# Tonmoy1321/Multimodal-DeepFake-Detection

Measured on AMD Instinct MI355X. Metric: clips/sec (node) XceptionLSTMV 16x299x299 bf16 train, higher is better.
Workload: dtype bf16; 1 GPU; XceptionLSTMV(hidden=128) unfrozen-backbone train step, 16 clips/GPU x 16 frames x 3x299x299, BCE + clip 1.0 + Adam; global_batch=16, frames=16, size=299, mode=unfrozen, optimizer=clip 1.0 + Adam, xcp FusedAdamClip, parallelism=dp1, execution=eager launches

## Files before the change

### include/xcp.h

```cpp
#ifndef XCP_H_
#define XCP_H_

#ifdef __cplusplus
extern "C" {
#endif

typedef void* xcp_stream_t;

#define XCP_OK 0
#define XCP_EINVAL 1001
#define XCP_EUNSUPPORTED 1002
#define XCP_F32 0
#define XCP_BF16 1
#define XCP_ACT_NONE 0
#define XCP_ACT_RELU 1
#define XCP_ACT_BNRELU 2

int xcp_gemm_nt(int dtype, const void* A, long lda, const void* B, long ldb, void* C, long ldc, int M, int N, int K,
                float* stats, int gmode, int gH, int gW, int gOH, int gOW, int gS, int gC, int tile, xcp_stream_t stream);
int xcp_gemm_nt_stat_rows(int M);

int xcp_gemm_tn_rows_per_split(int dtype, int gmode, int M, int N, int K, int tile);
int xcp_gemm_tn(int dtype, const void* G, long ldg, const void* X, long ldx, float* P, int M, int N, int K, int S,
                int rows_per_split, int gmode, int gH, int gW, int gOH, int gOW, int gS, int gC, int tile,
// ... 13 lines not shown
int xcp_dw_bwd(int dtype, int act, const void* dY, const void* X, const float* Wt, const float* scale, const float* shift,
               const void* dRes, const void* dSkip, int sOH, int sOW, int sS, int skip_pre, void* dX, float* dWpart,
               float* bnpart, const float* bmean, const float* binvstd, int N, int H, int W, int C,
               xcp_stream_t stream);
int xcp_dw_bwd_resbn(int dtype, int act, const void* dY, const void* X, const float* Wt, const float* scale,
                     const float* shift, const void* dRes, void* dX, float* dWpart, float* bnpart, const float* bmean,
                     const float* binvstd, const void* Yb, int N, int H, int W, int C, xcp_stream_t stream);

int xcp_colreduce_f32(const float* in, int S, long L, long ld, float* out, int G, int accumulate, xcp_stream_t stream);
int xcp_colreduce_multi(const long long* jobs, int njobs, xcp_stream_t stream);
int xcp_colreduce_groups(int S, long L);
int xcp_chanred_parts(long rows, int C);
int xcp_row_stats(int dtype, const void* X, long rows, int C, float* part, xcp_stream_t stream);
int xcp_bn_bwd_reduce(int dtype, const void* dZ, const void* Y, const float* mean, const float* invstd,
                      const float* ms, const float* mt, long rows, int C, float* part, xcp_stream_t stream);
int xcp_bn_finalize_part(const float* part, int R, int C, int CP, double count, const float* gamma, const float* beta,
                         float* rmean, float* rvar, float momentum, float eps, float* mean_o, float* invstd_o,
                         float* scale_o, float* shift_o, xcp_stream_t stream);
#define XCP_FIN_ACCUMULATE 1
#define XCP_FIN_NARROW 2
int xcp_bn_bwd_finalize_part(const float* part, int R, int C, int CP, double count, const float* gamma,
                             const float* mean, const float* invstd, float* alpha, float* bcoef, float* delta,
                             float* dgamma, float* dbeta, int flags, xcp_stream_t stream);
int xcp_bn_finalize(const double* part2, int G, int C, int CP, double count, const float* gamma, const float* beta,
                    float* rmean, float* rvar, float momentum, float eps, int train, float* mean, float* invstd,
                    float* scale, float* shift, xcp_stream_t stream);
int xcp_bn_act(int dtype, const void* X, void* Y, const float* scale, const float* shift, int relu, long rows, int C,
               xcp_stream_t stream);
int xcp_bn_act_strided(int dtype, const void* X, void* Y, const float* scale, const float* shift, int relu, int N, int H,
                       int W, int OH, int OW, int S, int C, xcp_stream_t stream);
int xcp_bn_bwd_apply(int dtype, const void* dZ, const void* Y, void* dY, const float* alpha, const float* bcoef,
                     const float* delta, const float* ms, const float* mt, long rows, int C, xcp_stream_t stream);
int xcp_relu_bwd(int dtype, void* dX, const void* X, long rows, int C, xcp_stream_t stream);
int xcp_tail_fwd(int dtype, const void* Y, const float* s1, const float* t1, int pool, const void* S, const float* s2,
                 const float* t2, void* Out, unsigned char* amax, int N, int H, int W, int C, xcp_stream_t stream);
int xcp_maxpool_bwd(int dtype, const void* dOut, const unsigned char* amax, void* dZ, int N, int H, int W, int C,
                    xcp_stream_t stream);
int xcp_maxpool_bwd_bnred_parts(int N, int H, int W, int C);
int xcp_maxpool_bwd_bnred(int dtype, const void* dOut, const unsigned char* amax, void* dZ, const void* Y,
                          const float* mean, const float* invstd, int N, int H, int W, int C, float* part,
                          xcp_stream_t stream);
int xcp_avgpool_fwd(int dtype, const void* Y, const float* s, const float* t, float* F, int N, int HW, int C,
                    xcp_stream_t stream);
int xcp_avgpool_bwd(int dtype, const float* dF, const void* Y, const float* s, const float* t, void* dZ, int N, int HW,
                    int C, xcp_stream_t stream);

int xcp_conv1_fwd(int dtype, const float* X, const float* W, void* Y, int N, int IH, int IW, xcp_stream_t stream);
// ... 63 lines not shown
```

### multimodal-deepfake-detection_amd/xcp/_lib.py

```python
import ctypes
import os

_HERE = os.path.dirname(os.path.abspath(__file__))
LIB_PATH = DEFAULT_LIB_PATH = os.path.join(_HERE, "libxcp.so")
_REPO = os.path.dirname(os.path.dirname(_HERE))
_OVERRIDE = os.environ.get("XCP_LIB_PATH")
if _OVERRIDE:
    _real = os.path.realpath(_OVERRIDE)
    if os.path.commonpath([_real, os.path.realpath(_REPO)]) != os.path.realpath(_REPO):
        raise ImportError(f"XCP_LIB_PATH={_OVERRIDE} is outside the repository ({_REPO}); "
                          "only in-tree A/B builds may replace libxcp.so")
    LIB_PATH = _real
MISSING = []

P = ctypes.c_void_p
I = ctypes.c_int
L = ctypes.c_long
F = ctypes.c_float
D = ctypes.c_double

SIGNATURES = {
    "xcp_gemm_nt": [I, P, L, P, L, P, L, I, I, I, P, I, I, I, I, I, I, I, I, P],
    "xcp_gemm_nt_stat_rows": [I],
    "xcp_gemm_tn_rows_per_split": [I, I, I, I, I, I],
    "xcp_gemm_tn": [I, P, L, P, L, P, I, I, I, I, I, I, I, I, I, I, I, I, I, P],
    "xcp_unit_bwd_rows_per_split": [I, I, I, I],
    "xcp_unit_bwd": [I, P, P, P, P, P, P, P, P, P, I, I, I, I, I, P],
    "xcp_dw_fwd": [I, I, P, P, P, P, P, I, I, I, I, P],
    "xcp_sep_fwd_parts": [I, I, I, I, I, I],
    "xcp_sep_fwd": [I, I, P, P, P, P, P, P, P, P, I, I, I, I, I, P],
    "xcp_dw_bwd_chunks": [I, I, I, I],
    "xcp_dw_bwd": [I, I, P, P, P, P, P, P, P, I, I, I, I, P, P, P, P, P, I, I, I, I, P],
    "xcp_dw_bwd_resbn": [I, I, P, P, P, P, P, P, P, P, P, P, P, P, I, I, I, I, P],
    "xcp_colreduce_f32": [P, I, L, L, P, I, I, P],
    "xcp_colreduce_groups": [I, L],
    "xcp_colreduce_multi": [P, I, P],
    "xcp_chanred_parts": [L, I],
    "xcp_row_stats": [I, P, L, I, P, P],
    "xcp_bn_bwd_reduce": [I, P, P, P, P, P, P, L, I, P, P],
    "xcp_bn_finalize_part": [P, I, I, I, D, P, P, P, P, F, F, P, P, P, P, P],
    "xcp_bn_bwd_finalize_part": [P, I, I, I, D, P, P, P, P, P, P, P, P, I, P],
    "xcp_bn_finalize": [P, I, I, I, D, P, P, P, P, F, F, I, P, P, P, P, P],
    "xcp_bn_act": [I, P, P, P, P, I, L, I, P],
    "xcp_bn_act_strided": [I, P, P, P, P, I, I, I, I, I, I, I, I, P],
    "xcp_bn_bwd_apply": [I, P, P, P, P, P, P, P, P, L, I, P],
    "xcp_relu_bwd": [I, P, P, L, I, P],
    "xcp_tail_fwd": [I, P, P, P, I, P, P, P, P, P, I, I, I, I, P],
    "xcp_maxpool_bwd": [I, P, P, P, I, I, I, I, P],
    "xcp_maxpool_bwd_bnred_parts": [I, I, I, I],
    "xcp_maxpool_bwd_bnred": [I, P, P, P, P, P, P, I, I, I, I, P, P],
    "xcp_avgpool_fwd": [I, P, P, P, P, I, I, I, P],
    "xcp_avgpool_bwd": [I, P, P, P, P, P, I, I, I, P],
    "xcp_conv1_fwd": [I, P, P, P, I, I, I, P],
    "xcp_conv1_fwd_parts": [I, I, I],
    "xcp_conv1_fwd_stats": [I, P, P, P, P, I, I, I, P],
    "xcp_conv1_wgrad_parts": [I, I, I],
    "xcp_conv1_wgrad": [I, P, P, P, I, I, I, P],
    "xcp_conv1_wgrad_fused": [I, I, I],
    "xcp_conv1_wgrad_bn": [I, P, P, P, P, P, P, P, P, P, I, I, I, P],
    "xcp_permute3": [I, P, P, I, I, I, I, I, I, P],
# ... 73 lines not shown
```

### multimodal-deepfake-detection_amd/xcp/csrc/bn.hip

```cpp
#include "common.h"

namespace {

template <bool ACC, int VEC>
__global__ __launch_bounds__(256) void colreduce_kernel(const float* __restrict__ in, int S, long L, long ld,
                                                        float* __restrict__ out, int G) {
  __shared__ double red[4][64 * VEC];
  const int lane = threadIdx.x & 63, w = threadIdx.x >> 6;
  const long col = ((long)blockIdx.x * 64 + lane) * VEC;
  const int g = blockIdx.y;
  const int spg = (S + G - 1) / G;
  const int s0 = g * spg, s1 = min(S, s0 + spg);
  double acc[VEC];
#pragma unroll
  for (int j = 0; j < VEC; ++j) acc[j] = 0.0;
  if (col < L) {
    const float* p = in + col;
    int s = s0 + w;
    for (; s + 12 < s1; s += 16) {
      float v[4][VEC];
#pragma unroll
      for (int u = 0; u < 4; ++u) VecIO<float, VEC>::load(p + (long)(s + 4 * u) * ld, v[u]);
#pragma unroll
      for (int u = 0; u < 4; ++u)
// ... 142 lines not shown
};

template <typename T, int CPT> struct RawVec;
template <> struct RawVec<bf16, 8> { typedef uint4 type; };
template <> struct RawVec<bf16, 4> { typedef uint2 type; };
template <> struct RawVec<bf16, 2> { typedef unsigned type; };
struct U4x2 { uint4 a, b; };
template <> struct RawVec<float, 8> { typedef U4x2 type; };
template <> struct RawVec<float, 4> { typedef uint4 type; };
template <> struct RawVec<float, 2> { typedef uint2 type; };
template <> struct RawVec<float, 1> { typedef unsigned type; };

template <typename T, int MODE, int CPT>
__global__ __launch_bounds__(256) void chanred_kernel(ChanRed r, const void* Av, const void* Bv, const float* mean,
                                                      const float* invstd, const float* ms, const float* mt,
                                                      float* part) {
  const int cchunk = blockIdx.x % r.nch, pchunk = blockIdx.x / r.nch;
  const int lcv = threadIdx.x % r.CVB, slot = threadIdx.x / r.CVB;
  const int cv = cchunk * r.CVB + lcv;
  const int c0 = cv * CPT;
  const T* A = reinterpret_cast<const T*>(Av);
  const T* B = reinterpret_cast<const T*>(Bv);
  float acc[2][CPT];
#pragma unroll
  for (int j = 0; j < CPT; ++j) acc[0][j] = acc[1][j] = 0.f;
  if (slot < r.SPB && cv < r.CV) {
    float mu[CPT], is[CPT], sm[CPT], tm[CPT];
    if constexpr (MODE >= 1) {
      VecIO<float, CPT>::load(mean + c0, mu);
      VecIO<float, CPT>::load(invstd + c0, is);
    }
    if constexpr (MODE == 2) {
      VecIO<float, CPT>::load(ms + c0, sm);
      VecIO<float, CPT>::load(mt + c0, tm);
    }
    const long rb = (long)pchunk * r.rows_per_chunk, re = min(r.rows, rb + r.rows_per_chunk);
    constexpr int CR_U = 8;
    constexpr int NB = MODE == 0 ? 1 : 2;
    typedef typename RawVec<T, CPT>::type RV;
    const unsigned last = (unsigned)(re - 1) * (unsigned)r.C + (unsigned)c0, ustep = (unsigned)r.SPB * (unsigned)r.C;
    for (long p0 = rb + slot; p0 < re; p0 += (long)CR_U * r.SPB) {
      RV raw[NB][CR_U];
      const unsigned o0 = (unsigned)p0 * (unsigned)r.C + (unsigned)c0;
#pragma unroll
      for (int u = 0; u < CR_U; ++u) {
        const unsigned o = min(o0 + (unsigned)u * ustep, last);
        raw[0][u] = *reinterpret_cast<const RV*>(A + o);
        if constexpr (MODE >= 1) raw[NB - 1][u] = *reinterpret_cast<const RV*>(B + o);
      }
      __builtin_amdgcn_sched_barrier(0);
#pragma unroll
      for (int u = 0; u < CR_U; ++u) {
        const bool ok = p0 + (long)u * r.SPB < re;
        float a[CPT];
        VecIO<T, CPT>::load(reinterpret_cast<const T*>(&raw[0][u]), a);
#pragma unroll
        for (int j = 0; j < CPT; ++j) a[j] = ok ? a[j] : 0.f;
        if constexpr (MODE == 0) {
#pragma unroll
          for (int j = 0; j < CPT; ++j) {
            acc[0][j] += a[j];
            acc[1][j] = fmaf(a[j], a[j], acc[1][j]);
          }
        } else {
          float b[CPT];
          VecIO<T, CPT>::load(reinterpret_cast<const T*>(&raw[NB - 1][u]), b);
          if constexpr (MODE == 2) {
#pragma unroll
            for (int j = 0; j < CPT; ++j) a[j] = fmaf(b[j], sm[j], tm[j]) > 0.f ? a[j] : 0.f;
          }
#pragma unroll
          for (int j = 0; j < CPT; ++j) {
            acc[0][j] += a[j];
            acc[1][j] = fmaf(a[j], (b[j] - mu[j]) * is[j], acc[1][j]);
          }
        }
      }
    }
  }
  chanred_finish<CPT>(r, acc, part, cchunk, pchunk, lcv, slot);
}

// ... 157 lines not shown
  const long n = p / ((long)OH * OW);
  const int rem = (int)(p - n * OH * OW), oh = rem / OW, ow = rem - oh * OW;
  const long q = (n * H + (long)oh * S) * W + (long)ow * S;
  float v[CPT], s[CPT], t[CPT];
  VecIO<T, CPT>::load(X + q * C + c0, v);
  VecIO<float, CPT>::load(scale + c0, s);
  VecIO<float, CPT>::load(shift + c0, t);
#pragma unroll
  for (int j = 0; j < CPT; ++j) {
    v[j] = fmaf(v[j], s[j], t[j]);
    if (relu) v[j] = fmaxf(v[j], 0.f);
  }
  VecIO<T, CPT>::store(Y + p * C + c0, v);
}

template <typename T, int CPT, bool MASK, int RPT>
__global__ __launch_bounds__(256) void bn_bwd_apply_kernel(const T* __restrict__ dZ, const T* __restrict__ Yv, T* dY,
                                                           const float* alpha, const float* bcoef, const float* delta,
                                                           const float* ms, const float* mt, long rows, int C) {
  const unsigned CV = (unsigned)C / CPT;
  const unsigned rq = (unsigned)((rows + RPT - 1) / RPT), nrows = (unsigned)rows;
  const unsigned g = blockIdx.x * 256u + threadIdx.x;
  if (g >= rq * CV) return;
  const unsigned p0 = g / CV, c0 = (g - p0 * CV) * CPT;
  const unsigned o0 = p0 * (unsigned)C + c0, ostep = rq * (unsigned)C, olast = (nrows - 1) * (unsigned)C + c0;
  float dz[RPT][CPT], y[RPT][CPT], al[CPT], bc[CPT], de[CPT];
#pragma unroll
  for (int k = 0; k < RPT; ++k) {
    const unsigned o = min(o0 + k * ostep, olast);
    VecIO<T, CPT>::load(dZ + o, dz[k]);
    VecIO<T, CPT>::load(Yv + o, y[k]);
  }
  VecIO<float, CPT>::load(alpha + c0, al);
  VecIO<float, CPT>::load(bcoef + c0, bc);
  VecIO<float, CPT>::load(delta + c0, de);
  if constexpr (MASK) {
    float sm[CPT], tm[CPT];
    VecIO<float, CPT>::load(ms + c0, sm);
    VecIO<float, CPT>::load(mt + c0, tm);
#pragma unroll
    for (int k = 0; k < RPT; ++k)
#pragma unroll
      for (int j = 0; j < CPT; ++j) dz[k][j] = fmaf(y[k][j], sm[j], tm[j]) > 0.f ? dz[k][j] : 0.f;
  }
#pragma unroll
  for (int k = 0; k < RPT; ++k) {
// ... 370 lines not shown
  float y[CPT], sc[CPT], sh[CPT], d[CPT];
  VecIO<T, CPT>::load(Y + p * C + c0, y);
  VecIO<float, CPT>::load(s + c0, sc);
  VecIO<float, CPT>::load(t + c0, sh);
  VecIO<float, CPT>::load(dF + (long)n * C + c0, d);
  const float inv = 1.f / (float)HW;
#pragma unroll
  for (int j = 0; j < CPT; ++j) y[j] = fmaf(y[j], sc[j], sh[j]) > 0.f ? d[j] * inv : 0.f;
  VecIO<T, CPT>::store(dZ + p * C + c0, y);
}

inline unsigned nblk(long n) { return (unsigned)((n + 255) / 256); }

template <typename T, int MODE>
int chanred_launch(long rows, int C, const void* A, const void* B, const float* mean, const float* invstd, float* part,
                   hipStream_t st, const float* ms = nullptr, const float* mt = nullptr) {
  constexpr int CPT = 8;
  if (rows * C >= 0x7fffffffL) return XCP_EUNSUPPORTED;
  ChanRed r = make_chanred(rows, C, CPT, 1024);
  const long P = chanred_P(r);
  const size_t smem = (size_t)r.SPB * 2 * r.CVB * CPT * sizeof(float);
  hipLaunchKernelGGL((chanred_kernel<T, MODE, CPT>), dim3((unsigned)(P * r.nch)), dim3(256), smem, st, r, A, B, mean,
                     invstd, ms, mt, part);
  return (int)hipGetLastError();
}

inline PoolSrc pool_src(const void* dOut, const unsigned char* amax, int H, int W) {
  return PoolSrc{dOut, amax, H, W, (H - 1) / 2 + 1, (W - 1) / 2 + 1};
}

}

extern "C" {

int xcp_colreduce_f32(const float* in, int S, long L, long ld, float* out, int G, int accumulate, hipStream_t st) {
  if (L <= 0) return XCP_OK;
  if (ld < L) return XCP_EINVAL;
  if (G > S) G = S;
// ... 61 lines not shown

int xcp_bn_bwd_reduce(int dtype, const void* dZ, const void* Y, const float* mean, const float* invstd, const float* ms,
                      const float* mt, long rows, int C, float* part, hipStream_t st) {
  if (C % 8) return XCP_EINVAL;
  if ((ms == nullptr) != (mt == nullptr)) return XCP_EINVAL;
  if (ms) {
    if (dtype == XCP_BF16) return chanred_launch<bf16, 2>(rows, C, dZ, Y, mean, invstd, part, st, ms, mt);
    if (dtype == XCP_F32) return chanred_launch<float, 2>(rows, C, dZ, Y, mean, invstd, part, st, ms, mt);
    return XCP_EUNSUPPORTED;
  }
  if (dtype == XCP_BF16) return chanred_launch<bf16, 1>(rows, C, dZ, Y, mean, invstd, part, st);
  if (dtype == XCP_F32) return chanred_launch<float, 1>(rows, C, dZ, Y, mean, invstd, part, st);
  return XCP_EUNSUPPORTED;
}

int xcp_bn_finalize_part(const float* part, int R, int C, int CP, double count, const float* gamma, const float* beta,
                         float* rmean, float* rvar, float momentum, float eps, float* mean_o, float* invstd_o,
                         float* scale_o, float* shift_o, hipStream_t st) {
  if (C <= 0) return XCP_OK;
  if (R <= 0 || CP < C) return XCP_EINVAL;
  hipLaunchKernelGGL(bn_finalize_part_kernel, dim3((CP + FIN_CH - 1) / FIN_CH), dim3(64 * FIN_WAVES), 0, st, part, R,
                     C, CP, count, gamma, beta, rmean, rvar, momentum, eps, mean_o, invstd_o, scale_o, shift_o);
  return (int)hipGetLastError();
}

int xcp_bn_bwd_finalize_part(const float* part, int R, int C, int CP, double count, const float* gamma,
                             const float* mean, const float* invstd, float* alpha, float* bcoef, float* delta,
                             float* dgamma, float* dbeta, int flags, hipStream_t st) {
  if (C <= 0) return XCP_OK;
  if (R <= 0 || CP < C) return XCP_EINVAL;
// ... 47 lines not shown
                       shift, relu, H, W, OH, OW, S, rows, C);
  else
    return XCP_EUNSUPPORTED;
  return (int)hipGetLastError();
}

int xcp_bn_bwd_apply(int dtype, const void* dZ, const void* Y, void* dY, const float* alpha, const float* bcoef,
                     const float* delta, const float* ms, const float* mt, long rows, int C, hipStream_t st) {
  if (C % 8) return XCP_EINVAL;
  if ((ms == nullptr) != (mt == nullptr)) return XCP_EINVAL;
  if (rows <= 0) return XCP_OK;
  if (rows * C >= 0x7fffffffL) return XCP_EUNSUPPORTED;
  const long rq4 = (rows + 3) / 4, rq2 = (rows + 1) / 2;
#define XCP_APPLY(TT, MK)                                                                                       \
  hipLaunchKernelGGL((bn_bwd_apply_kernel<TT, 8, MK, MK ? 4 : 2>), dim3(nblk((MK ? rq4 : rq2) * (C / 8))),    \
                     dim3(256), 0, st, (const TT*)dZ, (const TT*)Y, (TT*)dY, alpha, bcoef, delta, ms, mt, rows, C)
  if (dtype == XCP_BF16) {
    if (ms) XCP_APPLY(bf16, true);
    else XCP_APPLY(bf16, false);
  } else if (dtype == XCP_F32) {
    if (ms) XCP_APPLY(float, true);
    else XCP_APPLY(float, false);
  } else
#undef XCP_APPLY
    return XCP_EUNSUPPORTED;
  return (int)hipGetLastError();
}

int xcp_relu_bwd(int dtype, void* dX, const void* X, long rows, int C, hipStream_t st) {
  if (C % 8) return XCP_EINVAL;
  const unsigned g = nblk(rows * (C / 8));
  if (dtype == XCP_BF16)
    hipLaunchKernelGGL((relu_bwd_kernel<bf16, 8>), dim3(g), dim3(256), 0, st, (bf16*)dX, (const bf16*)X, rows, C);
  else if (dtype == XCP_F32)
    hipLaunchKernelGGL((relu_bwd_kernel<float, 8>), dim3(g), dim3(256), 0, st, (float*)dX, (const float*)X, rows, C);
  else
    return XCP_EUNSUPPORTED;
  return (int)hipGetLastError();
}
// ... 99 lines not shown
```

### multimodal-deepfake-detection_amd/xcp/csrc/dwconv.hip

```cpp
#include "common.h"
#include <stdlib.h>

namespace {

constexpr int SLICE = 64;
constexpr int NW = 16;
constexpr int SEGL = 5;

constexpr int FWD_MAXPX = 512;

struct TileGeo {
  int TH, TW, HP, WP, nth, ntw, nseg;
};

inline TileGeo tile_geo(int H, int W, int maxpx, int segl = SEGL) {
  TileGeo g;
  g.ntw = (W + 39) / 40;
  g.TW = (W + g.ntw - 1) / g.ntw;
  g.nseg = (g.TW + segl - 1) / segl;
  g.WP = g.nseg * segl + 2;
  int thmax = maxpx / g.WP - 2;
  if (thmax < 1) thmax = 1;
  g.nth = (H + thmax - 1) / thmax;
  g.TH = (H + g.nth - 1) / g.nth;
// ... 483 lines not shown
    is = R::load(a.binvstd + cc);
  }
  unsigned okm = 0;
#pragma unroll
  for (int k = 0; k < RS + 2; ++k) {
    const int col = x0 - 1 + k;
    okm |= (col >= 0 && col < a.W) ? (1u << k) : 0u;
  }
  const long fbase = (long)mp.n * a.H * a.W * a.C;
  auto frame_rsrc = [&](const void* t) {
    return __builtin_amdgcn_make_buffer_rsrc(const_cast<T*>(reinterpret_cast<const T*>(t) + fbase), (short)0,
                                             DW_BUF_RECORDS, DW_BUF_DWORD3);
  };
  const __amdgpu_buffer_rsrc_t X = frame_rsrc(a.X), G = frame_rsrc(a.dY);
  const __amdgpu_buffer_rsrc_t dRes = frame_rsrc(RES ? a.dRes : a.X);
  const T* dSkip = reinterpret_cast<const T*>(a.dSkip);
  T* dX = reinterpret_cast<T*>(a.dX) + fbase;
  const int lofs = sg * RS * SLICE + cl * 4;
  auto rd = [&](const char* row, int k) {
    if constexpr (ASMRD) return ring_u32(row + lofs + k * SLICE);
    else return *reinterpret_cast<const unsigned*>(row + lofs + k * SLICE);
  };
  auto fence = [&](auto& v) {
    if constexpr (ASMRD) ring_fence(v);
  };
  auto cvtg = [&](const char* row, V (&gy)[RS + 2]) {
    unsigned u[RS + 2];
#pragma unroll
    for (int k = 0; k < RS + 2; ++k) u[k] = rd(row, k);
    fence(u);
#pragma unroll
    for (int k = 0; k < RS + 2; ++k) gy[k] = R::unpack(u[k]);
  };
  auto sx = [&](int r) { return rx + (r % NS) * LROW; };
  auto sgs = [&](int r) { return rg + ((r + NSG) % NSG) * LROW; };
  auto sr = [&](int r) { return rres + (r % NS) * LROW; };
  constexpr int L = RES ? 6 : 4;
  auto step = [&](int h, const V (&g0)[RS + 2], const V (&g1)[RS + 2], V (&g2)[RS + 2]) {
    char* sxh = sx(h);
    char* srh = sr(h);
    vmwait<2 + (BD - 1) * (L + 2)>();
    const bool skip_row = SKIP && dSkip && (h % a.sS) == 0 && h / a.sS < a.sOH;
    unsigned pskp[RS];
#pragma unroll
    for (int j = 0; j < RS; ++j) pskp[j] = 0u;
    unsigned pyb[RES ? RS : 1];
    if constexpr (RES) {
      if constexpr (bnres) {
        const T* yrow = reinterpret_cast<const T*>(a.Yb) + fbase + (long)h * a.W * a.C + cc;
#pragma unroll
        for (int j = 0; j < RS; ++j) pyb[j] = *reinterpret_cast<const unsigned*>(yrow + (long)min(x0 + j, a.W - 1) * a.C);
      }
    }
    if constexpr (SKIP) {
      const int srow = min(h / a.sS, max(a.sOH - 1, 0));
#pragma unroll
      for (int j = 0; j < RS; ++j) {
        const int ow = x0 + j;
        const bool ok = skip_row && cok && ow % a.sS == 0 && ow / a.sS < a.sOW && ow < a.W;
        const int scol = min(max(ow, 0) / a.sS, max(a.sOW - 1, 0));
        const T* ptr = dSkip ? dSkip + (((long)mp.n * a.sOH + srow) * a.sOW + scol) * a.C + cc
                             : reinterpret_cast<const T*>(g_dzero);
        const unsigned v = *reinterpret_cast<const unsigned*>(ptr);
        pskp[j] = ok ? v : 0u;
      }
    }
// ... 53 lines not shown
        V gw[RS + 2];
        cvtg(sgs(h + 1 - ky), gw);
        if (ky == 2 && h == 0) {
#pragma unroll
          for (int k = 0; k < RS + 2; ++k) gw[k] = V(0.f);
        }
#pragma unroll
        for (int kx = 0; kx < 3; ++kx)
#pragma unroll
          for (int j = 0; j < RS; ++j) sj[j] = vfma(gw[j + 2 - kx], wt[ky * 3 + kx], sj[j]);
#pragma unroll
        for (int j = 0; j < RS; ++j)
#pragma unroll
          for (int kx = 0; kx < 3; ++kx) dw[ky * 3 + kx] = vfma(gw[j + 1], xa[j + kx], dw[ky * 3 + kx]);
      }
    }
#pragma unroll
    for (int j = 0; j < RS; ++j) {
      V s = sj[j];
      if (skip_row && a.skip_pre) s += R::unpack(pskp[j]);
      if constexpr (ACT != ACT_NONE) {
        const V ctr = xa[j + 1];
        if constexpr (EPT == 2) {
          s[0] = ctr[0] > 0.f ? s[0] : 0.f;
          s[1] = ctr[1] > 0.f ? s[1] : 0.f;
        } else {
          s = ctr > 0.f ? s : 0.f;
        }
      }
      if (bnx) {
// ... 240 lines not shown
```

### multimodal-deepfake-detection_amd/xcp/engine.py

```python
import contextlib
import os
import math

import torch
import torch.nn as nn

from . import ops
from .ops import ACT_BNRELU, ACT_NONE, ACT_RELU


def _bn_ref(m):
    return {"weight": m.weight, "bias": m.bias, "running_mean": m.running_mean, "running_var": m.running_var,
            "eps": m.eps, "momentum": m.momentum, "track": m.track_running_stats, "module": m}


class _Unit:

    def __init__(self, sep, bn, relu, name, bn_name):
        self.sep, self.bn, self.relu, self.name, self.bn_name = sep, bn, relu, name, bn_name
        self.cin = sep.conv1.in_channels
        self.cout = sep.pointwise.out_channels
        if sep.conv1.kernel_size != (3, 3) or sep.conv1.stride != (1, 1) or sep.conv1.padding != (1, 1):
            raise NotImplementedError("xcp engine supports the Xception 3x3/s1/p1 separable convs only")
        if sep.conv1.bias is not None or sep.pointwise.bias is not None:
# ... 41 lines not shown

class Stats:
    __slots__ = ("mean", "invstd", "scale", "shift")

    def __init__(self, C, dev):
        buf = torch.empty(4 * C, device=dev, dtype=torch.float32)
        self.mean, self.invstd, self.scale, self.shift = buf[:C], buf[C:2 * C], buf[2 * C:3 * C], buf[3 * C:]

    def __getitem__(self, k):
        return getattr(self, k)


WGRAD_SIDE_STREAM = os.environ.get("XCP_WGRAD_STREAM", "1") != "0"
FUSED_UNIT_BWD = os.environ.get("XCP_FUSED_UNIT_BWD", "1") != "0"
STEM_FUSED = os.environ.get("XCP_STEM_FUSED", "1") != "0"
RESBN = os.environ.get("XCP_RESBN", "0") == "1"
STEM_WGRAD_SIDE = WGRAD_SIDE_STREAM and os.environ.get("XCP_STEM_WGRAD_SIDE", "1") != "0"
SIDE_PRIO_LOW = os.environ.get("XCP_SIDE_PRIO", "") == "low"
STEM_BN1_FIRST = os.environ.get("XCP_STEM_BN1_FIRST", "1") != "0"
CONV1_BN_FUSED = os.environ.get("XCP_CONV1_BN_FUSED", "1") != "0"
STEM_WGRAD_EARLY = os.environ.get("XCP_STEM_WGRAD_EARLY", "1") != "0"
STEM_FIN_NARROW = os.environ.get("XCP_STEM_FIN_NARROW", "1") != "0"
CONV1_STATS_FUSED = os.environ.get("XCP_CONV1_STATS_FUSED", "1") != "0"
DW_REDUCE_SIDE = WGRAD_SIDE_STREAM and os.environ.get("XCP_DW_REDUCE_SIDE", "1") != "0"
REDUCE_BATCH = os.environ.get("XCP_REDUCE_BATCH", "1") != "0"
SEP_FUSED = os.environ.get("XCP_SEP_FUSED", "1") != "0"
SEP_MIN_W = {128: 0, 256: 0} if os.environ.get("XCP_SEP_NARROW", "0") == "1" else {128: 120, 256: 64}
CONV2_ACT_ON_LOAD = os.environ.get("XCP_CONV2_ACTIN", "1") != "0"
WGRAD_FIRST = os.environ.get("XCP_WGRAD_FIRST", "0") == "1"
WGRAD_DEFER = os.environ.get("XCP_WGRAD_DEFER", "0") == "1"
SKIP_WGRAD_LATE = os.environ.get("XCP_SKIP_WGRAD_LATE", "0") == "1"
# ... 335 lines not shown
                deferred.clear()

        def done():
            flush_deferred()
            if rbatch is not None and rbatch.jobs:
                if side is not None:
                    side.wait_stream(main)
                    with torch.cuda.stream(side):
                        rbatch.flush()
                else:
                    rbatch.flush()
            if notify is not None and pending:
                notify(list(pending), side)
            pending.clear()

        def bn_coef(bnmod, name, dZ, Y, rows, C, st, part=None, relu=False, narrow=False):
            P = part[1] if part is not None else 0
            (gw, acc), (gb, acc_b) = g(name + ".weight", (C,)), g(name + ".bias", (C,))
            if acc != acc_b:
                raise NotImplementedError(f"xcp engine: {name}.weight and .bias must both (or neither) require grad")
            return ops.bn_backward_coef(dZ, Y, rows, C, _bn_ref(bnmod), st, gw, gb,
                                        part=part[0] if part is not None else None, R=P, relu=relu, accumulate=acc,
                                        CP=pc(C), narrow=narrow)

        def bn_bwd(bnmod, name, dZ, Y, rows, C, st, part=None, relu=False):
            coef = bn_coef(bnmod, name, dZ, Y, rows, C, st, part, relu)
            dY = self._empty(rows * pc(C))
            ops.bn_apply_coef(dZ, Y, dY, coef, st, rows, pc(C), relu)
            return dY

        def unit_bwd(u, rec, dZ, H, W, dRes=None, dSkip=None, skip_geom=(0, 0, 1), part=None, prev_st=None,
                     skip_pre=False, res_bn=None):
            M = N * H * W
            dD = self._empty(M * pc(u.cin))
            if FUSED_UNIT_BWD and ops.unit_bwd_rows_per_split(dZ.dtype, M, u.cout, u.cin) > 0:
                coef = bn_coef(u.bn, u.bn_name, dZ, rec["y"], M, u.cout, rec["st"], part)
                dst, acc = g(u.name + ".pointwise.weight", (u.cout, u.cin, 1, 1))
                ops.unit_bwd(dZ, rec["y"], coef, pk[u.name + ".pwT"], rec["d"], dD, M, u.cout, u.cin, dst, acc)
            else:
                dY = bn_bwd(u.bn, u.bn_name, dZ, rec["y"], M, u.cout, rec["st"], part)
                if WGRAD_FIRST:
                    wgrad(dY, rec["d"], M, u.cout, u.cin, u.name + ".pointwise.weight", (u.cout, u.cin, 1, 1))
                ops.gemm_nt(dY, pk[u.name + ".pwT"], dD, M, pc(u.cin), pc(u.cout), tile=NT_TILE)
                if not WGRAD_FIRST:
                    wgrad(dY, rec["d"], M, u.cout, u.cin, u.name + ".pointwise.weight", (u.cout, u.cin, 1, 1),
                          defer=WGRAD_DEFER)
            dX = self._empty(M * pc(u.cin))
            dwg, acc = g(u.name + ".conv1.weight", (u.cin, 1, 3, 3))
            bnp = ops.dw_bwd(rec["act"], dD, rec["src"], pk[u.name + ".dw"], rec["sc"], rec["sh"], dX, dwg, N, H, W,
                             pc(u.cin), dRes=dRes, dSkip=dSkip, skip_geom=skip_geom,
                             bn_stats=res_bn[1] if res_bn is not None else prev_st, accumulate=acc,
                             Cw=u.cin, skip_pre=skip_pre, reduce_stream=side if DW_REDUCE_SIDE else None,
                             keep=keep, batch=rbatch, res_bn_input=res_bn[0] if res_bn is not None else None)
            return dX, (bnp if prev_st is not None or res_bn is not None else None)

        H, W = S["xH"], S["xW"]
        M = N * H * W
        e3, e4 = S["exit"]
        u3, u4 = self.exit_units
        dZ4 = self._empty(M * 2048)
        ops.avgpool_bwd(dfeat, e4["y"], e4["st"].scale, e4["st"].shift, dZ4, N, H * W, 2048)
        dZ3, p3 = unit_bwd(u4, e4, dZ4, H, W, prev_st=e3["st"])
        dX, _ = unit_bwd(u3, e3, dZ3, H, W, part=p3)
        done()
        pre_part = part_in = None
        for k in range(len(self.blocks) - 1, -1, -1):
            prev = (self.blocks[k - 1], S["blocks"][k - 1]) if k > 0 else None
            dX, pre_part, part_in = self._block_bwd(self.blocks[k], S["blocks"][k], dX, N, pk, bn_bwd, unit_bwd,
                                                    wgrad, part_in, prev)
            done()
        OH1, OW1, OH2, OW2 = S["OH1"], S["OW1"], S["OH2"], S["OW2"]
        rows1, rows2 = N * OH1 * OW1, N * OH2 * OW2
        if pre_part is not None:
            dC2 = bn_bwd(m.bn2, "bn2", dX, S["c2"], rows2, 64, S["s2"], part=pre_part)
        else:
            dC2 = bn_bwd(m.bn2, "bn2", dX, S["c2"], rows2, 64, S["s2"], relu=True)
        def conv2_wgrad(st2):
# ... 130 lines not shown
```

### multimodal-deepfake-detection_amd/xcp/ops.py

```python
import torch

from . import _lib

F32, BF16 = 0, 1
ACT_NONE, ACT_RELU, ACT_BNRELU = 0, 1, 2
DT = {torch.float32: F32, torch.bfloat16: BF16}


def _p(t):
    return 0 if t is None else t.data_ptr()


def stream():
    return torch.cuda.current_stream().cuda_stream


def device_guard(t):
    return torch.cuda.device(t.device)


class KernelTimer:

    def __init__(self, classes):
        self.classes = classes
# ... 223 lines not shown


def eval_stats(C, bn, out, device, CP=None):
    p2 = torch.zeros(2 * (CP or C), device=device, dtype=torch.float64)
    _bn_finalize(p2, 1, C, 1.0, bn, False, out, CP)


def row_stats(X, rows, C):
    R = _lib.call("xcp_chanred_parts", rows, C)
    part = torch.empty(R * 2 * C, device=X.device, dtype=torch.float32)
    _lib.call("xcp_row_stats", DT[X.dtype], _p(X), rows, C, _p(part), stream())
    return part, R


def bn_backward_coef(dZ, Y, rows, C, bn, st, dgamma, dbeta, part=None, R=0, relu=False, accumulate=False, CP=None,
                     narrow=False):
    CP = CP or C
    ms, mt = (_p(st["scale"]), _p(st["shift"])) if relu else (0, 0)
    dev, dt = Y.device, Y.dtype
    if part is None:
        R = _lib.call("xcp_chanred_parts", rows, CP)
        part = torch.empty(R * 2 * CP, device=dev, dtype=torch.float32)
        _lib.call("xcp_bn_bwd_reduce", DT[dt], _p(dZ), _p(Y), _p(st["mean"]), _p(st["invstd"]), ms, mt, rows, CP,
                  _p(part), stream())
    elif relu:
        raise ValueError("a fused partial cannot carry the ReLU mask")
    coef = torch.empty(3 * CP, device=dev, dtype=torch.float32)
    part, R = _fold(part, R, CP)
    _lib.call("xcp_bn_bwd_finalize_part", _p(part), R, C, CP, float(rows), _p(bn["weight"]), _p(st["mean"]),
              _p(st["invstd"]), _p(coef), _p(coef[CP:]), _p(coef[2 * CP:]), _p(dgamma), _p(dbeta),
              (1 if accumulate else 0) | (2 if narrow else 0), stream())
    return coef


def bn_backward(dZ, Y, rows, C, bn, st, dY, dgamma, dbeta, part=None, R=0, relu=False, accumulate=False):
    coef = bn_backward_coef(dZ, Y, rows, C, bn, st, dgamma, dbeta, part=part, R=R, relu=relu, accumulate=accumulate)
    bn_apply_coef(dZ, Y, dY, coef, st, rows, C, relu)


def bn_apply_coef(dZ, Y, dY, coef, st, rows, C, relu=False):
    ms, mt = (_p(st["scale"]), _p(st["shift"])) if relu else (0, 0)
    _lib.call("xcp_bn_bwd_apply", DT[Y.dtype], _p(dZ), _p(Y), _p(dY), _p(coef), _p(coef[C:]), _p(coef[2 * C:]), ms,
              mt, rows, C, stream())


def unit_bwd_rows_per_split(dtype, M, CO, CI):
    return _lib.call("xcp_unit_bwd_rows_per_split", DT[dtype], M, CO, CI)


def unit_bwd(G, Y, coef, Wt, X, dD, M, CO, CI, dW_out, accumulate=False):
    rps = unit_bwd_rows_per_split(G.dtype, M, CO, CI)
    if rps <= 0:
        raise ValueError(f"xcp.unit_bwd: unsupported shape M={M} CO={CO} CI={CI} dtype={G.dtype}")
    S = (M + rps - 1) // rps
    P = torch.empty(S * CO * CI, device=G.device, dtype=torch.float32)
    with _timed("unit_bwd", {"M": M, "CO": CO, "CI": CI}):
# ... 201 lines not shown
```

Before: 443.9 clips/s.

## Fuse exit avgpool backward into BN backward via broadcast gradient; enable RESBN by default

The exit block no longer materializes the full-resolution dZ4 tensor from the pooled gradient. New MODE=3 channel reduction and broadcast apply kernels read the fp32 pooled gradient per sample, divide by HW and apply the ReLU mask from Y. The change also switches the residual-BN backward path on by default and moves its Y loads in the depthwise backward kernel to buffer loads staged through LDS. It is meant to save one full 2048-channel tensor write and read plus a kernel launch, at the cost of more kernel variants and a changed load schedule in the dwconv kernel.

Result: no change. 446.1 clips/s, median of 6 (+0.5%).

```diff
diff --git a/include/xcp.h b/include/xcp.h
--- a/include/xcp.h
+++ b/include/xcp.h
@@ -51,6 +51,8 @@
 int xcp_row_stats(int dtype, const void* X, long rows, int C, float* part, xcp_stream_t stream);
 int xcp_bn_bwd_reduce(int dtype, const void* dZ, const void* Y, const float* mean, const float* invstd,
                       const float* ms, const float* mt, long rows, int C, float* part, xcp_stream_t stream);
+int xcp_bn_bwd_reduce_bcast(int dtype, const float* dF, int HW, const void* Y, const float* mean, const float* invstd,
+                            const float* ms, const float* mt, long rows, int C, float* part, xcp_stream_t stream);
 int xcp_bn_finalize_part(const float* part, int R, int C, int CP, double count, const float* gamma, const float* beta,
                          float* rmean, float* rvar, float momentum, float eps, float* mean_o, float* invstd_o,
                          float* scale_o, float* shift_o, xcp_stream_t stream);
@@ -68,6 +70,9 @@
                        int W, int OH, int OW, int S, int C, xcp_stream_t stream);
 int xcp_bn_bwd_apply(int dtype, const void* dZ, const void* Y, void* dY, const float* alpha, const float* bcoef,
                      const float* delta, const float* ms, const float* mt, long rows, int C, xcp_stream_t stream);
+int xcp_bn_bwd_apply_bcast(int dtype, const float* dF, int HW, const void* Y, void* dY, const float* alpha,
+                           const float* bcoef, const float* delta, const float* ms, const float* mt, long rows, int C,
+                           xcp_stream_t stream);
 int xcp_relu_bwd(int dtype, void* dX, const void* X, long rows, int C, xcp_stream_t stream);
 int xcp_tail_fwd(int dtype, const void* Y, const float* s1, const float* t1, int pool, const void* S, const float* s2,
                  const float* t2, void* Out, unsigned char* amax, int N, int H, int W, int C, xcp_stream_t stream);
diff --git a/multimodal-deepfake-detection_amd/xcp/_lib.py b/multimodal-deepfake-detection_amd/xcp/_lib.py
--- a/multimodal-deepfake-detection_amd/xcp/_lib.py
+++ b/multimodal-deepfake-detection_amd/xcp/_lib.py
@@ -38,12 +38,14 @@
     "xcp_chanred_parts": [L, I],
     "xcp_row_stats": [I, P, L, I, P, P],
     "xcp_bn_bwd_reduce": [I, P, P, P, P, P, P, L, I, P, P],
+    "xcp_bn_bwd_reduce_bcast": [I, P, I, P, P, P, P, P, L, I, P, P],
     "xcp_bn_finalize_part": [P, I, I, I, D, P, P, P, P, F, F, P, P, P, P, P],
     "xcp_bn_bwd_finalize_part": [P, I, I, I, D, P, P, P, P, P, P, P, P, I, P],
     "xcp_bn_finalize": [P, I, I, I, D, P, P, P, P, F, F, I, P, P, P, P, P],
     "xcp_bn_act": [I, P, P, P, P, I, L, I, P],
     "xcp_bn_act_strided": [I, P, P, P, P, I, I, I, I, I, I, I, I, P],
     "xcp_bn_bwd_apply": [I, P, P, P, P, P, P, P, P, L, I, P],
+    "xcp_bn_bwd_apply_bcast": [I, P, I, P, P, P, P, P, P, P, L, I, P],
     "xcp_relu_bwd": [I, P, P, L, I, P],
     "xcp_tail_fwd": [I, P, P, P, I, P, P, P, P, P, I, I, I, I, P],
     "xcp_maxpool_bwd": [I, P, P, P, I, I, I, I, P],
diff --git a/multimodal-deepfake-detection_amd/xcp/csrc/bn.hip b/multimodal-deepfake-detection_amd/xcp/csrc/bn.hip
--- a/multimodal-deepfake-detection_amd/xcp/csrc/bn.hip
+++ b/multimodal-deepfake-detection_amd/xcp/csrc/bn.hip
@@ -180,7 +180,7 @@
 template <typename T, int MODE, int CPT>
 __global__ __launch_bounds__(256) void chanred_kernel(ChanRed r, const void* Av, const void* Bv, const float* mean,
                                                       const float* invstd, const float* ms, const float* mt,
-                                                      float* part) {
+                                                      float* part, int bhw) {
   const int cchunk = blockIdx.x % r.nch, pchunk = blockIdx.x / r.nch;
   const int lcv = threadIdx.x % r.CVB, slot = threadIdx.x / r.CVB;
   const int cv = cchunk * r.CVB + lcv;
@@ -196,22 +196,31 @@
       VecIO<float, CPT>::load(mean + c0, mu);
       VecIO<float, CPT>::load(invstd + c0, is);
     }
-    if constexpr (MODE == 2) {
+    if constexpr (MODE >= 2) {
       VecIO<float, CPT>::load(ms + c0, sm);
       VecIO<float, CPT>::load(mt + c0, tm);
     }
+    const float binv = 1.f / (float)bhw;
     const long rb = (long)pchunk * r.rows_per_chunk, re = min(r.rows, rb + r.rows_per_chunk);
-    constexpr int CR_U = 8;
+    constexpr int CR_U = MODE == 3 ? 4 : 8;
     constexpr int NB = MODE == 0 ? 1 : 2;
     typedef typename RawVec<T, CPT>::type RV;
+    typedef typename RawVec<float, CPT>::type RVF;
     const unsigned last = (unsigned)(re - 1) * (unsigned)r.C + (unsigned)c0, ustep = (unsigned)r.SPB * (unsigned)r.C;
     for (long p0 = rb + slot; p0 < re; p0 += (long)CR_U * r.SPB) {
       RV raw[NB][CR_U];
+      RVF braw[MODE == 3 ? CR_U : 1];
       const unsigned o0 = (unsigned)p0 * (unsigned)r.C + (unsigned)c0;
 #pragma unroll
       for (int u = 0; u < CR_U; ++u) {
         const unsigned o = min(o0 + (unsigned)u * ustep, last);
-        raw[0][u] = *reinterpret_cast<const RV*>(A + o);
+        if constexpr (MODE == 3) {
+          const unsigned row = min((unsigned)p0 + (unsigned)u * (unsigned)r.SPB, (unsigned)(re - 1));
+          braw[u] = *reinterpret_cast<const RVF*>(reinterpret_cast<const float*>(Av) + row / (unsigned)bhw * (unsigned)r.C +
+                                                  (unsigned)c0);
+        } else {
+          raw[0][u] = *reinterpret_cast<const RV*>(A + o);
+        }
         if constexpr (MODE >= 1) raw[NB - 1][u] = *reinterpret_cast<const RV*>(B + o);
       }
       __builtin_amdgcn_sched_barrier(0);
@@ -219,7 +228,13 @@
       for (int u = 0; u < CR_U; ++u) {
         const bool ok = p0 + (long)u * r.SPB < re;
         float a[CPT];
-        VecIO<T, CPT>::load(reinterpret_cast<const T*>(&raw[0][u]), a);
+        if constexpr (MODE == 3) {
+          VecIO<float, CPT>::load(reinterpret_cast<const float*>(&braw[u]), a);
+#pragma unroll
+          for (int j = 0; j < CPT; ++j) a[j] = rnd<T>(__fmul_rn(a[j], binv));
+        } else {
+          VecIO<T, CPT>::load(reinterpret_cast<const T*>(&raw[0][u]), a);
+        }
 #pragma unroll
         for (int j = 0; j < CPT; ++j) a[j] = ok ? a[j] : 0.f;
         if constexpr (MODE == 0) {
@@ -231,7 +246,7 @@
         } else {
           float b[CPT];
           VecIO<T, CPT>::load(reinterpret_cast<const T*>(&raw[NB - 1][u]), b);
-          if constexpr (MODE == 2) {
+          if constexpr (MODE >= 2) {
 #pragma unroll
             for (int j = 0; j < CPT; ++j) a[j] = fmaf(b[j], sm[j], tm[j]) > 0.f ? a[j] : 0.f;
           }
@@ -419,10 +434,12 @@
   VecIO<T, CPT>::store(Y + p * C + c0, v);
 }
 
-template <typename T, int CPT, bool MASK, int RPT>
-__global__ __launch_bounds__(256) void bn_bwd_apply_kernel(const T* __restrict__ dZ, const T* __restrict__ Yv, T* dY,
+template <typename T, int CPT, bool MASK, int RPT, bool BCAST = false>
+__global__ __launch_bounds__(256) void bn_bwd_apply_kernel(const void* __restrict__ dZv, const T* __restrict__ Yv, T* dY,
                                                            const float* alpha, const float* bcoef, const float* delta,
-                                                           const float* ms, const float* mt, long rows, int C) {
+                                                           const float* ms, const float* mt, long rows, int C, int bhw) {
+  static_assert(MASK || !BCAST, "the broadcast gradient is that of relu(bn(y))");
+  const T* dZ = reinterpret_cast<const T*>(dZv);
   const unsigned CV = (unsigned)C / CPT;
   const unsigned rq = (unsigned)((rows + RPT - 1) / RPT), nrows = (unsigned)rows;
   const unsigned g = blockIdx.x * 256u + threadIdx.x;
@@ -433,8 +450,20 @@
 #pragma unroll
   for (int k = 0; k < RPT; ++k) {
     const unsigned o = min(o0 + k * ostep, olast);
-    VecIO<T, CPT>::load(dZ + o, dz[k]);
+    if constexpr (BCAST) {
+      const unsigned row = min(p0 + k * rq, nrows - 1);
+      VecIO<float, CPT>::load(reinterpret_cast<const float*>(dZv) + row / (unsigned)bhw * (unsigned)C + c0, dz[k]);
+    } else {
+      VecIO<T, CPT>::load(dZ + o, dz[k]);
+    }
     VecIO<T, CPT>::load(Yv + o, y[k]);
+  }
+  if constexpr (BCAST) {
+    const float binv = 1.f / (float)bhw;
+#pragma unroll
+    for (int k = 0; k < RPT; ++k)
+#pragma unroll
+      for (int j = 0; j < CPT; ++j) dz[k][j] = rnd<T>(__fmul_rn(dz[k][j], binv));
   }
   VecIO<float, CPT>::load(alpha + c0, al);
   VecIO<float, CPT>::load(bcoef + c0, bc);
@@ -835,14 +864,14 @@
 
 template <typename T, int MODE>
 int chanred_launch(long rows, int C, const void* A, const void* B, const float* mean, const float* invstd, float* part,
-                   hipStream_t st, const float* ms = nullptr, const float* mt = nullptr) {
+                   hipStream_t st, const float* ms = nullptr, const float* mt = nullptr, int bhw = 1) {
   constexpr int CPT = 8;
   if (rows * C >= 0x7fffffffL) return XCP_EUNSUPPORTED;
   ChanRed r = make_chanred(rows, C, CPT, 1024);
   const long P = chanred_P(r);
   const size_t smem = (size_t)r.SPB * 2 * r.CVB * CPT * sizeof(float);
   hipLaunchKernelGGL((chanred_kernel<T, MODE, CPT>), dim3((unsigned)(P * r.nch)), dim3(256), smem, st, r, A, B, mean,
-                     invstd, ms, mt, part);
+                     invstd, ms, mt, part, bhw);
   return (int)hipGetLastError();
 }
 
@@ -934,6 +963,14 @@
   return XCP_EUNSUPPORTED;
 }
 
+int xcp_bn_bwd_reduce_bcast(int dtype, const float* dF, int HW, const void* Y, const float* mean, const float* invstd,
+                            const float* ms, const float* mt, long rows, int C, float* part, hipStream_t st) {
+  if (C % 8 || HW <= 0 || rows % HW || !ms || !mt) return XCP_EINVAL;
+  if (dtype == XCP_BF16) return chanred_launch<bf16, 3>(rows, C, dF, Y, mean, invstd, part, st, ms, mt, HW);
+  if (dtype == XCP_F32) return chanred_launch<float, 3>(rows, C, dF, Y, mean, invstd, part, st, ms, mt, HW);
+  return XCP_EUNSUPPORTED;
+}
+
 int xcp_bn_finalize_part(const float* part, int R, int C, int CP, double count, const float* gamma, const float* beta,
                          float* rmean, float* rvar, float momentum, float eps, float* mean_o, float* invstd_o,
                          float* scale_o, float* shift_o, hipStream_t st) {
@@ -1011,7 +1048,7 @@
   const long rq4 = (rows + 3) / 4, rq2 = (rows + 1) / 2;
 #define XCP_APPLY(TT, MK)                                                                                       \
   hipLaunchKernelGGL((bn_bwd_apply_kernel<TT, 8, MK, MK ? 4 : 2>), dim3(nblk((MK ? rq4 : rq2) * (C / 8))),    \
-                     dim3(256), 0, st, (const TT*)dZ, (const TT*)Y, (TT*)dY, alpha, bcoef, delta, ms, mt, rows, C)
+                     dim3(256), 0, st, dZ, (const TT*)Y, (TT*)dY, alpha, bcoef, delta, ms, mt, rows, C, 1)
   if (dtype == XCP_BF16) {
     if (ms) XCP_APPLY(bf16, true);
     else XCP_APPLY(bf16, false);
@@ -1020,6 +1057,24 @@
     else XCP_APPLY(float, false);
   } else
 #undef XCP_APPLY
+    return XCP_EUNSUPPORTED;
+  return (int)hipGetLastError();
+}
+
+int xcp_bn_bwd_apply_bcast(int dtype, const float* dF, int HW, const void* Y, void* dY, const float* alpha,
+                           const float* bcoef, const float* delta, const float* ms, const float* mt, long rows, int C,
+                           hipStream_t st) {
+  if (C % 8 || HW <= 0 || rows % HW || !ms || !mt) return XCP_EINVAL;
+  if (rows <= 0) return XCP_OK;
+  if (rows * C >= 0x7fffffffL) return XCP_EUNSUPPORTED;
+  const unsigned g = nblk((rows + 3) / 4 * (C / 8));
+  if (dtype == XCP_BF16)
+    hipLaunchKernelGGL((bn_bwd_apply_kernel<bf16, 8, true, 4, true>), dim3(g), dim3(256), 0, st, dF, (const bf16*)Y,
+                       (bf16*)dY, alpha, bcoef, delta, ms, mt, rows, C, HW);
+  else if (dtype == XCP_F32)
+    hipLaunchKernelGGL((bn_bwd_apply_kernel<float, 8, true, 4, true>), dim3(g), dim3(256), 0, st, dF, (const float*)Y,
+                       (float*)dY, alpha, bcoef, delta, ms, mt, rows, C, HW);
+  else
     return XCP_EUNSUPPORTED;
   return (int)hipGetLastError();
 }
diff --git a/multimodal-deepfake-detection_amd/xcp/csrc/dwconv.hip b/multimodal-deepfake-detection_amd/xcp/csrc/dwconv.hip
--- a/multimodal-deepfake-detection_amd/xcp/csrc/dwconv.hip
+++ b/multimodal-deepfake-detection_amd/xcp/csrc/dwconv.hip
@@ -521,6 +521,7 @@
   };
   const __amdgpu_buffer_rsrc_t X = frame_rsrc(a.X), G = frame_rsrc(a.dY);
   const __amdgpu_buffer_rsrc_t dRes = frame_rsrc(RES ? a.dRes : a.X);
+  const __amdgpu_buffer_rsrc_t Yb = frame_rsrc(bnres ? a.Yb : a.X);
   const T* dSkip = reinterpret_cast<const T*>(a.dSkip);
   T* dX = reinterpret_cast<T*>(a.dX) + fbase;
   const int lofs = sg * RS * SLICE + cl * 4;
@@ -543,20 +544,22 @@
   auto sgs = [&](int r) { return rg + ((r + NSG) % NSG) * LROW; };
   auto sr = [&](int r) { return rres + (r % NS) * LROW; };
   constexpr int L = RES ? 6 : 4;
+  constexpr int YB = bnres ? 2 : 0;
   auto step = [&](int h, const V (&g0)[RS + 2], const V (&g1)[RS + 2], V (&g2)[RS + 2]) {
     char* sxh = sx(h);
     char* srh = sr(h);
-    vmwait<2 + (BD - 1) * (L + 2)>();
+    vmwait<2 + (BD - 1) * (YB + L + 2)>();
     const bool skip_row = SKIP && dSkip && (h % a.sS) == 0 && h / a.sS < a.sOH;
     unsigned pskp[RS];
 #pragma unroll
     for (int j = 0; j < RS; ++j) pskp[j] = 0u;
-    unsigned pyb[RES ? RS : 1];
-    if constexpr (RES) {
-      if constexpr (bnres) {
-        const T* yrow = reinterpret_cast<const T*>(a.Yb) + fbase + (long)h * a.W * a.C + cc;
-#pragma unroll
-        for (int j = 0; j < RS; ++j) pyb[j] = *reinterpret_cast<const unsigned*>(yrow + (long)min(x0 + j, a.W - 1) * a.C);
+    dwu4 yv[2];
+    if constexpr (bnres) {
+      const unsigned rowb = (unsigned)(h * a.W * a.C * (int)sizeof(T));
+#pragma unroll
+      for (int i = 0; i < 2; ++i) {
+        const int o = rl_st.off[i] >= 0 ? (int)(rowb + (unsigned)(rl_st.off[i] * (int)sizeof(T))) : (int)DW_BUF_OOB;
+        yv[i] = __builtin_bit_cast(dwu4, __builtin_amdgcn_raw_buffer_load_b128(Yb, o, 0, 0));
       }
     }
     if constexpr (SKIP) {
@@ -640,6 +643,20 @@
 #pragma unroll
           for (int kx = 0; kx < 3; ++kx) dw[ky * 3 + kx] = vfma(gw[j + 1], xa[j + kx], dw[ky * 3 + kx]);
       }
+    }
+    unsigned pyb[RES ? RS : 1];
+    if constexpr (bnres) {
+      __builtin_amdgcn_sched_barrier(0);
+      const char* ych[2] = {stg + lane * 16, stg + (lane < 4 * RCOLS - 64 ? 64 + lane : lane) * 16};
+#pragma unroll
+      for (int i = 1; i >= 0; --i)
+        asm volatile("ds_write_b128 %0, %1"
+                     :
+                     : "v"((unsigned)(size_t)(const __attribute__((address_space(3))) char*)(ych[i])), "v"(yv[i])
+                     : "memory");
+#pragma unroll
+      for (int j = 0; j < RS; ++j) pyb[j] = ring_u32(stg + (sg * RS + j) * SLICE + cl * 4);
+      ring_fence(pyb);
     }
 #pragma unroll
     for (int j = 0; j < RS; ++j) {
diff --git a/multimodal-deepfake-detection_amd/xcp/engine.py b/multimodal-deepfake-detection_amd/xcp/engine.py
--- a/multimodal-deepfake-detection_amd/xcp/engine.py
+++ b/multimodal-deepfake-detection_amd/xcp/engine.py
@@ -79,7 +79,8 @@
 WGRAD_SIDE_STREAM = os.environ.get("XCP_WGRAD_STREAM", "1") != "0"
 FUSED_UNIT_BWD = os.environ.get("XCP_FUSED_UNIT_BWD", "1") != "0"
 STEM_FUSED = os.environ.get("XCP_STEM_FUSED", "1") != "0"
-RESBN = os.environ.get("XCP_RESBN", "0") == "1"
+RESBN = os.environ.get("XCP_RESBN", "1") != "0"
+EXIT_BCAST = os.environ.get("XCP_EXIT_BCAST", "1") != "0"
 STEM_WGRAD_SIDE = WGRAD_SIDE_STREAM and os.environ.get("XCP_STEM_WGRAD_SIDE", "1") != "0"
 SIDE_PRIO_LOW = os.environ.get("XCP_SIDE_PRIO", "") == "low"
 STEM_BN1_FIRST = os.environ.get("XCP_STEM_BN1_FIRST", "1") != "0"
@@ -445,31 +446,34 @@
                 notify(list(pending), side)
             pending.clear()
 
-        def bn_coef(bnmod, name, dZ, Y, rows, C, st, part=None, relu=False, narrow=False):
+        def bn_coef(bnmod, name, dZ, Y, rows, C, st, part=None, relu=False, narrow=False, bcast_hw=0):
             P = part[1] if part is not None else 0
             (gw, acc), (gb, acc_b) = g(name + ".weight", (C,)), g(name + ".bias", (C,))
             if acc != acc_b:
                 raise NotImplementedError(f"xcp engine: {name}.weight and .bias must both (or neither) require grad")
             return ops.bn_backward_coef(dZ, Y, rows, C, _bn_ref(bnmod), st, gw, gb,
                                         part=part[0] if part is not None else None, R=P, relu=relu, accumulate=acc,
-                                        CP=pc(C), narrow=narrow)
-
-        def bn_bwd(bnmod, name, dZ, Y, rows, C, st, part=None, relu=False):
-            coef = bn_coef(bnmod, name, dZ, Y, rows, C, st, part, relu)
+                                        CP=pc(C), narrow=narrow, bcast_hw=bcast_hw)
+
+        def bn_bwd(bnmod, name, dZ, Y, rows, C, st, part=None, relu=False, bcast_hw=0):
+            coef = bn_coef(bnmod, name, dZ, Y, rows, C, st, part, relu, bcast_hw=bcast_hw)
             dY = self._empty(rows * pc(C))
-            ops.bn_apply_coef(dZ, Y, dY, coef, st, rows, pc(C), relu)
+            ops.bn_apply_coef(dZ, Y, dY, coef, st, rows, pc(C), relu, bcast_hw=bcast_hw)
             return dY
 
         def unit_bwd(u, rec, dZ, H, W, dRes=None, dSkip=None, skip_geom=(0, 0, 1), part=None, prev_st=None,
-                     skip_pre=False, res_bn=None):
+                     skip_pre=False, res_bn=None, pool_hw=0):
             M = N * H * W
             dD = self._empty(M * pc(u.cin))
-            if FUSED_UNIT_BWD and ops.unit_bwd_rows_per_split(dZ.dtype, M, u.cout, u.cin) > 0:
+            if not pool_hw and FUSED_UNIT_BWD and ops.unit_bwd_rows_per_split(dZ.dtype, M, u.cout, u.cin) > 0:
                 coef = bn_coef(u.bn, u.bn_name, dZ, rec["y"], M, u.cout, rec["st"], part)
                 dst, acc = g(u.name + ".pointwise.weight", (u.cout, u.cin, 1, 1))
                 ops.unit_bwd(dZ, rec["y"], coef, pk[u.name + ".pwT"], rec["d"], dD, M, u.cout, u.cin, dst, acc)
             else:
-                dY = bn_bwd(u.bn, u.bn_name, dZ, rec["y"], M, u.cout, rec["st"], part)
+                if pool_hw:
+                    dY = bn_bwd(u.bn, u.bn_name, dZ, rec["y"], M, u.cout, rec["st"], relu=True, bcast_hw=pool_hw)
+                else:
+                    dY = bn_bwd(u.bn, u.bn_name, dZ, rec["y"], M, u.cout, rec["st"], part)
                 if WGRAD_FIRST:
                     wgrad(dY, rec["d"], M, u.cout, u.cin, u.name + ".pointwise.weight", (u.cout, u.cin, 1, 1))
                 ops.gemm_nt(dY, pk[u.name + ".pwT"], dD, M, pc(u.cin), pc(u.cout), tile=NT_TILE)
@@ -489,9 +493,12 @@
         M = N * H * W
         e3, e4 = S["exit"]
         u3, u4 = self.exit_units
-        dZ4 = self._empty(M * 2048)
-        ops.avgpool_bwd(dfeat, e4["y"], e4["st"].scale, e4["st"].shift, dZ4, N, H * W, 2048)
-        dZ3, p3 = unit_bwd(u4, e4, dZ4, H, W, prev_st=e3["st"])
+        if EXIT_BCAST:
+            dZ3, p3 = unit_bwd(u4, e4, dfeat, H, W, prev_st=e3["st"], pool_hw=H * W)
+        else:
+            dZ4 = self._empty(M * 2048)
+            ops.avgpool_bwd(dfeat, e4["y"], e4["st"].scale, e4["st"].shift, dZ4, N, H * W, 2048)
+            dZ3, p3 = unit_bwd(u4, e4, dZ4, H, W, prev_st=e3["st"])
         dX, _ = unit_bwd(u3, e3, dZ3, H, W, part=p3)
         done()
         pre_part = part_in = None
diff --git a/multimodal-deepfake-detection_amd/xcp/ops.py b/multimodal-deepfake-detection_amd/xcp/ops.py
--- a/multimodal-deepfake-detection_amd/xcp/ops.py
+++ b/multimodal-deepfake-detection_amd/xcp/ops.py
@@ -261,11 +261,18 @@
 
 
 def bn_backward_coef(dZ, Y, rows, C, bn, st, dgamma, dbeta, part=None, R=0, relu=False, accumulate=False, CP=None,
-                     narrow=False):
+                     narrow=False, bcast_hw=0):
     CP = CP or C
     ms, mt = (_p(st["scale"]), _p(st["shift"])) if relu else (0, 0)
     dev, dt = Y.device, Y.dtype
-    if part is None:
+    if bcast_hw:
+        if part is not None or not relu or CP != C or dZ.dtype != torch.float32:
+            raise ValueError("xcp.bn_backward_coef: a broadcast gradient is fp32, of relu(bn(Y)), at pitch C, unreduced")
+        R = _lib.call("xcp_chanred_parts", rows, CP)
+        part = torch.empty(R * 2 * CP, device=dev, dtype=torch.float32)
+        _lib.call("xcp_bn_bwd_reduce_bcast", DT[dt], _p(dZ), bcast_hw, _p(Y), _p(st["mean"]), _p(st["invstd"]), ms, mt,
+                  rows, CP, _p(part), stream())
+    elif part is None:
         R = _lib.call("xcp_chanred_parts", rows, CP)
         part = torch.empty(R * 2 * CP, device=dev, dtype=torch.float32)
         _lib.call("xcp_bn_bwd_reduce", DT[dt], _p(dZ), _p(Y), _p(st["mean"]), _p(st["invstd"]), ms, mt, rows, CP,
@@ -285,8 +292,14 @@
     bn_apply_coef(dZ, Y, dY, coef, st, rows, C, relu)
 
 
-def bn_apply_coef(dZ, Y, dY, coef, st, rows, C, relu=False):
+def bn_apply_coef(dZ, Y, dY, coef, st, rows, C, relu=False, bcast_hw=0):
     ms, mt = (_p(st["scale"]), _p(st["shift"])) if relu else (0, 0)
+    if bcast_hw:
+        if not relu or dZ.dtype != torch.float32:
+            raise ValueError("xcp.bn_apply_coef: a broadcast gradient is fp32 and that of relu(bn(Y))")
+        _lib.call("xcp_bn_bwd_apply_bcast", DT[Y.dtype], _p(dZ), bcast_hw, _p(Y), _p(dY), _p(coef), _p(coef[C:]),
+                  _p(coef[2 * C:]), ms, mt, rows, C, stream())
+        return
     _lib.call("xcp_bn_bwd_apply", DT[Y.dtype], _p(dZ), _p(Y), _p(dY), _p(coef), _p(coef[C:]), _p(coef[2 * C:]), ms,
               mt, rows, C, stream())
 
```
